# TAMS-Group/bio_ik

Hardware: AMD Instinct MI355X
Metric: IK solves/sec (pop=128, 7-DOF PoseGoal batch) (higher is better)
Workload: dtype f64

## Files before the change

bio_ik_amd/csrc/bioik_kernels.h:

```cpp
#pragma once
#include <type_traits>

#include "bioik_device.h"


#ifndef BIOIK_CANDIDATE_BOUND
#define BIOIK_CANDIDATE_BOUND BIOIK_SINCOS_DOMAIN
#endif
#ifndef BIOIK_COOP_WALKS
#define BIOIK_COOP_WALKS 1
#endif

struct LdsLayout {
    int seed, par, pop, sol, prefix, state, clip, xcol, slots, g_first, g_stride, total;
    int xn, gv, frames, tips, delta, base, grad, red, sec, order, bc;
    int xm, xp, dv, fc;
    int fitp;
    int help;
};
BIOIK_HD LdsLayout make_layout(int n_ops, int V, int P, int T, int n_slots, int nthreads, int lambda, int has_secondary, int child_cols = 1,
                               int groups = 1, int slot_sets = 1, int fit_park = 0, int fc_in_pop = 0, int helped = 0, int bounded = 0) {
    LdsLayout L;
    const int m = n_ops > 0 ? n_ops : 1;
    int o = 0;
// ... 624 lines not shown
        }
    }
    template <class Fn>
    BIOIK_DEV double group_value(bool glead, int gtid, double* s_bc, Fn&& fn) {
        double v = 0.0;
        if (glead) v = fn();
        if (G > 64) {
            if (gtid == 0) s_bc[0] = v;
            wg_barrier();
            v = s_bc[0];
            wg_barrier();
        }
        return v;
    }
    BIOIK_DEV FitCheck group_check(bool glead, int gtid, double* s_bc, const XV& x) {
        const QueryCtx qc{s_seed, s_par};
        FitCheck fc{0.0, 0};
        if (glead) {
            if (BIOIK_COOP_WALKS == 0) fc = exact_fitness_check(pb, x, qc, s_slots, sp.dpos, sp.drot, sp.dtwist, 1, s_prefix);
            else if (G >= 64) fc = exact_fitness_check<64>(pb, x, qc, s_slots, sp.dpos, sp.drot, sp.dtwist, 1, s_prefix);
            else fc = exact_fitness_check<32>(pb, x, qc, s_slots, sp.dpos, sp.drot, sp.dtwist, 1, s_prefix);
        }
        if (G > 64) {
            if (gtid == 0) s_bc[0] = fc.fitness, s_bc[2] = (double)fc.ok;
            wg_barrier();
            fc.fitness = s_bc[0];
            fc.ok = (int)s_bc[2];
            wg_barrier();
        }
        return fc;
    }
    BIOIK_DEV FitCheck wg_check(bool wlead, int tid, const XV& x, double dpos, double drot, double dtwist, int do_check) {
        const QueryCtx qc{s_seed, s_par};
        FitCheck fc{0.0, 0};
        if (wlead) fc = exact_fitness_check<BIOIK_COOP_WALKS ? 64 : 0>(pb, x, qc, s_slots, dpos, drot, dtwist, do_check, s_prefix);
        if (nth > 64) {
            double* const s_wbc = s_state + 16;
            if (tid == 0) s_wbc[0] = fc.fitness, s_wbc[1] = (double)fc.ok;
            wg_barrier();
            fc.fitness = s_wbc[0];
            fc.ok = (int)s_wbc[1];
            wg_barrier();
        }
        return fc;
    }
    BIOIK_DEV SpeciesState species_load(int r) const {
        const double* d = s_state + r * 8;
        return SpeciesState{d[0], d[1], d[2], (int)d[3], (int)d[4], (int)d[5], (int)d[6], (int)d[7]};
    }
    BIOIK_DEV void species_store(int r, const SpeciesState& S) const {
        double* d = s_state + r * 8;
        d[0] = S.fit, d[1] = S.pf0, d[2] = S.pf1, d[3] = (double)S.id, d[4] = (double)S.slot, d[5] = (double)S.cur, d[6] = (double)S.improved, d[7] = (double)S.ok;
    }
    BIOIK_DEV int rank_now(int rank_it) const {
        return (SLIM && groups == 2) ? (HALVES ? p_lane_fresh() >> 5 : (WAVE2 ? p_wave_index() : (g_shift >= 0 ? p_tid_fresh() >> g_shift : p_tid_fresh() / G))) : rank_it;
    }
};

#if defined(BIOIK_PHASE_TIMING)
#define BIOIK_FRAME_PHASE_NAMES(F) auto& ph_t_ = (F).ph_t_; auto& ph_last_ = (F).ph_last_; auto& ph_start_ = (F).ph_start_;
#else
#define BIOIK_FRAME_PHASE_NAMES(F)
#endif
#define BIOIK_FRAME_NAMES(F)                                                                                                                                          \
    typedef typename Frame::PB PB;                                                                                                                                    \
    constexpr bool LEAN = Frame::LEAN, CL = Frame::CL, JOINT = Frame::JOINT, SLIM = Frame::SLIM, DENSE = Frame::DENSE, HELPED = Frame::HELPED, WAVE2 = Frame::WAVE2,   \
                   LIN = Frame::LIN, JH = Frame::JH, HALVES = Frame::HALVES, SELECTS = Frame::SELECTS, columnless = Frame::CL;                                        \
    constexpr int FIXED = Frame::FIXED;                                                                                                                               \
    const SolveArgs& a = (F).a;                                                                                                                                       \
    const DevSolveParams& sp = (F).sp;                                                                                                                                \
    double* const lds = (F).lds;                                                                                                                                      \
    const PB pb = (F).pb;                                                                                                                                             \
    const uint64_t unit = (F).unit, q = (F).q, active_mask = (F).active_mask;                                                                                         \
    const uint32_t key = (F).key;                                                                                                                                     \
    const bool resume = (F).resume, has_sec = (F).has_sec, exact = (F).exact, child_pairs = (F).child_pairs;                                                          \
    const int tid0 = (F).tid0, nth = (F).nth, V = (F).V, P = (F).P, T = (F).T, n_ops = (F).n_ops, D = (F).D, lambda = (F).lambda,                                     \
              n_cols = (F).n_cols, groups = (F).groups, G = (F).G, g_shift = (F).g_shift;                                                                             \
    const int M = n_ops > 0 ? n_ops : 1;                                                                                                                              \
    const int SP = 2 * 2 * 2 * M;                                                                                                   \
    const int BF = 4 * M;                                                             \
    const int carry_n = carry_doubles(n_ops);                                                                        \
    const LdsLayout& L = (F).L;                                                                                                                                       \
    double* const s_seed = (F).s_seed;                                                                                                                                \
    double* const s_par = (F).s_par;                                                                                                                                  \
    double* const s_pop = (F).s_pop;                                                                                                                                  \
    double* const s_sol = (F).s_sol;                                                                                                                                  \
    double* const s_prefix = (F).s_prefix;                                                                                                                            \
    double* const s_state = (F).s_state;                                                                                                                              \
    double* const s_slots = (F).s_slots;                                                                                                                              \
    double* const s_clip = (F).s_clip;                                                                                                                                \
    double* const s_wbc = s_state + 16;                                                                                          \
    double* const s_solst = s_state + 20;                                                                   \
    double* const s_deadline = s_state + 22;                   \
    const QueryCtx qc{s_seed, s_par};                                                                                                                                 \
    auto wg_barrier = [&]() { (F).wg_barrier(); };                                                                                                                    \
    auto species_load = [&](int r_) { return (F).species_load(r_); };                                                                                                 \
    auto species_store = [&](int r_, const SpeciesState& S_) { (F).species_store(r_, S_); };                                                                          \
    auto my_resident = [&]() { return (F).my_resident(); };                                                                                                           \
    (void)wg_barrier, (void)species_load, (void)species_store, (void)my_resident;                                               \
    BIOIK_FRAME_PHASE_NAMES(F)
template <class Frame>
BIOIK_DEV bool solve_setup(Frame& F, uint64_t unit_in) {
    typedef typename Frame::PB PB;
    constexpr bool LEAN = Frame::LEAN, CL = Frame::CL, SLIM = Frame::SLIM, DENSE = Frame::DENSE, HELPED = Frame::HELPED, WAVE2 = Frame::WAVE2, LIN = Frame::LIN, JH = Frame::JH, HALVES = Frame::HALVES;
    constexpr bool columnless = CL;
    constexpr int FIXED = Frame::FIXED;
// ... 564 lines not shown
    } else if (!JOINT && columnless) {
        for (int r = gtid; r < n_eval; r += G) {
            const int c = has_sec ? s_order[r] : r;
            const auto cx = make_child_x(pb, key, ctr1, (uint32_t)c + 2u, p0g, p0d, p1d);
            PHASE_MARK(PH_REPRODUCE);
            const double f = exact ? eval_exact_primary(pb, cx, qc, s_slots, s_prefix) : eval_linear_primary(pb, cx, qc, lm);
            PHASE_MARK(PH_FITNESS);
            offer(f, r + 2);
        }
    } else {
        for (int r = gtid, j = 0; r < n_eval; r += G, j++) {
            int c = has_sec ? s_order[r] : r;
            double* xc = stored ? xcol + (size_t)j * M * nth : xcol;
            const XV xv{xc, nth};
            reproduce_child(pb, key, ctr1, (uint32_t)c + 2u, p0g, p0d, p1d, xc, nth, nullptr, 0);
            PHASE_MARK(PH_REPRODUCE);
            double f = exact ? eval_exact_primary(pb, xv, qc, s_slots, s_prefix) : eval_linear_primary(pb, xv, qc, lm);
            PHASE_MARK(PH_FITNESS);
            offer(f, r + 2);
        }
    }
}

template <class Frame>
BIOIK_DEV void solve_select_and_copy(Frame& F, SpeciesState& S, double*& popS, int rank_it, int step, int gen, uint32_t ctr1, int n_eval, double& b1f, int& b1p, double& b2f, int& b2p) {
    BIOIK_FRAME_NAMES(F);
    auto rank_now = [&]() { return F.rank_now(rank_it); };
    BIOIK_LANE_SCOPE;
    const double* cb = popS + S.cur * BF;
    const double *p0g = cb, *p0d = cb + M, *p1d = cb + 3 * M;
    const bool stored = !columnless && n_cols * G >= lambda && (LEAN || pb->n_quat == 0);
    auto offer = [&](double f, int pos) { top2_insert(b1f, b1p, b2f, b2p, f, pos); };
    auto coarse_parked = [&](int gt) {
        if constexpr (SLIM && CL) {
            if (const int tie_bits = a.preselect >> 8) {
                double* const s_fq = gbase + L.fitp;
                for (int r = gt; r < n_eval; r += G) {
                    unsigned long long v;
                    __builtin_memcpy(&v, &s_fq[r], 8);
                    v &= ~((1ull << tie_bits) - 1ull);
                    __builtin_memcpy(&s_fq[r], &v, 8);
                }
                group_sync(G);
            }
        }
    };
    if constexpr (SLIM) S = species_load(rank_now()), popS = s_pop + S.slot * SP, cb = popS + S.cur * BF, p0g = cb, p0d = cb + M, p1d = cb + 3 * M;
    const uint32_t ctr1w = SLIM ? rng_ctr1((uint32_t)step * 16u + (uint32_t)gen, (uint32_t)S.id, RNG_REPRODUCE) : ctr1;
    if constexpr (DENSE || JH) coarse_parked(gtid);
    if constexpr (DENSE || JH) {
        const double* const s_fit2 = gbase + L.fitp;
        const int drop = a.sort_key_drop;
        unsigned long long k1 = ~0ull, k2 = ~0ull;
        for (int r = gtid; r < n_eval; r += G) {
            const unsigned long long k = sort_key(s_fit2[r], r + 2, drop);
            const bool w1 = k < k1, w2 = k < k2;
            k2 = w1 ? k1 : (w2 ? k : k2);
            k1 = w1 ? k : k1;
        }
        const unsigned long long B1 = half_min_u64(k1);
        const unsigned long long B2 = half_min_u64(k1 == B1 ? k2 : k1);
        int shares = 0;
        for (int r = gtid; r < n_eval; r += G) shares += ((sort_key(s_fit2[r], r + 2, drop) ^ B2) >> drop) == 0ull ? 1 : 0;
        const unsigned long long one = p_ballot(shares > 0), more = p_ballot(shares > 1);
        const uint32_t mine = grp ? (uint32_t)(one >> 32) : (uint32_t)one;
        const bool in_doubt = B2 != ~0ull && ((mine & (mine - 1u)) != 0u);
        if (p_ballot(in_doubt) == 0ull && more == 0ull) {
            b1p = (int)(B1 & 1023ull), b1f = s_fit2[b1p - 2];
            if (B2 != ~0ull) b2p = (int)(B2 & 1023ull), b2f = s_fit2[b2p - 2];
        } else {
            for (int r = gtid; r < n_eval; r += G) offer(s_fit2[r], r + 2);
            top2_wave(b1f, b1p, b2f, b2p, G);
        }
    } else {
        top2_wave(b1f, b1p, b2f, b2p, G);
    }
    PHASE_MARK(PH_SEL_TOP2);
    top2_xwave(b1f, b1p, b2f, b2p, s_red, gtid, G);
    PHASE_MARK(PH_SEL_XWAVE);
    if constexpr (SELECTS) {
        if (has_sec) {
            double* const s_fv = gbase + L.fitp;
            int t1 = 0, t2 = 0;
            for (int r = gtid; r < n_eval; r += G) {
                const double v = s_fv[r];
                t1 += v == b1f ? 1 : 0, t2 += v == b2f ? 1 : 0;
            }
            const unsigned long long gm = G >= 64 ? ~0ull : 0xffffffffull << (tid & 32);
            const unsigned long long o1 = p_ballot(t1 > 0) & gm, o2 = p_ballot(t2 > 0) & gm;
            const bool tie = (p_ballot(t1 > 1 || t2 > 1) & gm) != 0ull || (o1 & (o1 - 1ull)) != 0ull || (o2 & (o2 - 1ull)) != 0ull || (b2p != 0x7fffffff && b2f == S.pf0);
            if (p_ballot(tie) != 0ull) {
                auto stable_first = [&](double fwant, int skip, double& wf, int& wc) -> int {
                    double bs = P_INF;
                    int bc = 0x7fffffff, br = 0x7fffffff;
                    for (int r = gtid; r < n_eval; r += G) {
                        if (!(s_fv[r] == fwant) || r == skip) continue;
                        const int c = s_order[r];
                        const double sec = secondary_fitness<true>(pb, make_child_x(pb, key, ctr1w, (uint32_t)c + 2u, p0g, p0d, p1d), qc);
                        if (sec < bs || (sec == bs && c < bc)) bs = sec, bc = c, br = r;
                    }
                    double w2f = P_INF;
                    int w2c = 0x7fffffff;
                    wf = bs, wc = bc;
                    top2_wave(wf, wc, w2f, w2c, G);
                    const unsigned long long own = p_ballot(bc == wc && bc != 0x7fffffff) & gm;
                    const int src = own != 0ull ? __builtin_ctzll(own) : (tid & 63);
                    const int rr = p_shfl(br, src);
                    return own != 0ull ? rr : 0x7fffffff;
                };
                double e1, e2;
                int c1, c2;
                const int r1 = stable_first(b1f, -1, e1, c1);
                const int r2 = stable_first(b2f, r1, e2, c2);
                if (tie && r1 != 0x7fffffff) {
                    b1p = r1 + 2;
                    if (b2p != 0x7fffffff && r2 != 0x7fffffff) {
                        b2p = r2 + 2;
                        const bool first_is_first = e1 < e2 || (e1 == e2 && c1 < c2);
                        if (first_is_first != (r1 < r2)) {
                            if (gtid == 0) {
                                const int ca = s_order[r1], cb2 = s_order[r2];
                                const double fa = s_fv[r1], fb = s_fv[r2];
                                s_order[r1] = cb2, s_order[r2] = ca, s_fv[r1] = fb, s_fv[r2] = fa;
                            }
                            b1p = r2 + 2, b2p = r1 + 2;
                        }
                    }
                }
                group_sync(G);
            }
        }
    }
    Cand first{S.pf0, 0, 0};
    if (cand_better(S.pf1, 1, first.f, first.pos)) first = Cand{S.pf1, 1, 1};
    if (cand_better(b1f, b1p, first.f, first.pos)) first = Cand{b1f, b1p, b1p};
    const double c2f = (b1p == first.id) ? b2f : b1f;
    const int c2p = (b1p == first.id) ? b2p : b1p;
    Cand second{P_INF, 0x7fffffff, -1};
    if (first.id != 0) second = Cand{S.pf0, first.pos, 0};
    if (first.id != 1 && (second.id < 0 || cand_better(S.pf1, 1, second.f, second.pos))) second = Cand{S.pf1, 1, 1};
    if (second.id < 0 || cand_better(c2f, c2p, second.f, second.pos)) second = Cand{c2f, c2p, c2p};
    double* nb = popS + (S.cur ^ 1) * BF;
    const bool both_at_once = G >= 64 || M <= 16;
    for (int pass = 0; pass < (both_at_once ? 1 : 2); pass++) {
        BIOIK_LANE_SCOPE;
        if (gtid >= 64) break;
        const int i = G >= 64 ? gtid >> 5 : (both_at_once ? gtid >> 4 : pass), k0 = G >= 64 || !both_at_once ? gtid & 31 : gtid & 15;
        const int id = i == 0 ? first.id : second.id;
        double* dst = nb + i * 2 * M;
        if (id < 2) {
            const double* src = cb + id * 2 * M;
            if (k0 < M) dst[k0] = src[k0], dst[M + k0] = src[M + k0];
            if (M > 32 && k0 + 32 < M) dst[k0 + 32] = src[k0 + 32], dst[M + k0 + 32] = src[M + k0 + 32];
        } else if (stored) {
            BIOIK_FP_STRICT
            const int r = id - 2;
            const int c = has_sec ? s_order[r] : r;
            const double fmix = (((uint32_t)c + 2u) % 2u == 0u) ? 0.2 : 0.0;
            const int r_col = (G & (G - 1)) == 0 ? r >> (31 - __builtin_clz((unsigned)G)) : r / G, r_lane = r - r_col * G;
            const double* src = (lds + L.xcol) + (size_t)r_col * M * nth + (grp * G + r_lane);
            auto take = [&](int k) {
                double gene = src[(size_t)k * nth];
                double mom = 0.0;
                if ((active_mask >> k) & 1ull) {
                    double parent_gradient = p0d[k] * (1.0 - fmix) + p1d[k] * fmix;
                    mom = parent_gradient * (1.0 - 0.3) + (gene - p0g[k]) * 0.3;
                }
                dst[k] = gene, dst[M + k] = mom;
            };
            if (k0 < n_ops) take(k0);
            if (n_ops > 32 && k0 + 32 < n_ops) take(k0 + 32);
        } else if (LEAN) {
            BIOIK_FP_STRICT
            const int c = has_sec ? s_order[id - 2] : id - 2;
            const ChildX<PB> cx = make_child_x(pb, key, ctr1w, (uint32_t)c + 2u, p0g, p0d, p1d);
            auto derive = [&](int k) {
                const double gene = cx.template value<false>(k);
                double mom = 0.0;
                if ((active_mask >> k) & 1ull) {
                    const double parent_gradient = p0d[k] * (1.0 - cx.fmix) + p1d[k] * cx.fmix;
                    mom = parent_gradient * (1.0 - 0.3) + (gene - p0g[k]) * 0.3;
                }
                dst[k] = gene, dst[M + k] = mom;
            };
            if (k0 < n_ops) derive(k0);
            if (n_ops > 32 && k0 + 32 < n_ops) derive(k0 + 32);
        } else if (k0 == 0) {
            int c = has_sec ? s_order[id - 2] : id - 2;
            reproduce_child(pb, key, ctr1, (uint32_t)c + 2u, p0g, p0d, p1d, dst, 1, dst + M, 1);
        }
    }
    S.cur ^= 1;
    S.pf0 = first.f;
    S.pf1 = second.f;
    if constexpr (SLIM)
        if (gtid == 0) species_store(rank_now(), S);
    group_sync(G);
    PHASE_MARK(PH_SEL_COPY);
    group_sync(G);
    PHASE_MARK(PH_SEL_BAR);
}

template <class Frame>
BIOIK_DEV void solve_generation(Frame& F, SpeciesState& S, double*& popS, int rank_it, int step, int gen) {
    BIOIK_FRAME_NAMES(F);
    auto rank_now = [&]() { return F.rank_now(rank_it); };
    BIOIK_LANE_SCOPE;
    if constexpr (SLIM) S = species_load(rank_now()), popS = s_pop + S.slot * SP;
    const double* cb = popS + S.cur * BF;
    const double *p0g = cb, *p0d = cb + M, *p1d = cb + 3 * M;
    const uint32_t gctr = (uint32_t)step * 16u + (uint32_t)gen;
    const uint32_t ctr1 = rng_ctr1(gctr, (uint32_t)S.id, RNG_REPRODUCE);
    int n_eval = lambda;
    uint64_t inside_mask = 0ull;
    if constexpr (DENSE || WAVE2 || JH) {
        double* const pgt = popS + (S.cur ^ 1) * BF;
        bool inside = false;
        for (int k = gtid; k < n_ops; k += G) {
            const double d0 = p0d[k], d1 = p1d[k];
            const double pg0 = child_parent_gradient(d0, d1, 0), pg1 = child_parent_gradient(d0, d1, 1);
            pgt[k] = pg0, pgt[M + k] = pg1;
            if constexpr (WAVE2)
                inside = pb->ops[k].gene >= 0 && !op_unbounded(pb, k) && avoid_limits_surely_free(p0g[k], pg0, pg1, op_limit<LIM_VMIN>(pb, k), op_limit<LIM_VMAX>(pb, k), op_limit<LIM_SPAN>(pb, k));
        }
        if constexpr (WAVE2) inside_mask = has_sec ? p_ballot(inside) : 0ull;
        group_sync(G);
    }
    if (has_sec) solve_preselect(F, S, popS, step, gen, ctr1, inside_mask, n_eval);
    double b1f = P_INF, b2f = P_INF;
    int b1p = 0x7fffffff, b2p = 0x7fffffff;
    solve_walks(F, S, popS, rank_it, step, gen, ctr1, n_eval, b1f, b1p, b2f, b2p);
    solve_select_and_copy(F, S, popS, rank_it, step, gen, ctr1, n_eval, b1f, b1p, b2f, b2p);
}

template <class Frame>
BIOIK_DEV void solve_memetic(Frame& F, SpeciesState& S, double*& popS, int rank_it, int step) {
    BIOIK_FRAME_NAMES(F);
    auto rank_now = [&]() { return F.rank_now(rank_it); };
    if constexpr (SLIM) S = species_load(rank_now()), popS = s_pop + S.slot * SP;
    if (sp.memetic) {
        BIOIK_LANE_SCOPE;
        double* el = popS + S.cur * BF;
        const XV xe{el, 1};
        if (exact) build_approximator<BIOIK_COOP_WALKS>(pb, xe, s_slots, s_frames, s_tips, s_delta, s_base, gtid, G, s_prefix);
        PHASE_MARK(PH_MEM_APPROX);
        if (gtid < 64) {
            const int Gw = G < 64 ? G : 64;
            double dp = 0.0000001;
            {
                uint32_t o0, o1;
                philox2x32_10(key, rng_ctr0(0, 0), rng_ctr1((uint32_t)step * 16u, (uint32_t)S.id, RNG_MEMETIC_SIGN), o0, o1);
                if (rng_uniform(o0, o1) < 0.5) dp = -dp;
            }
            const bool by_op = pb_flavour<PB>::general ? pb->genes_follow_ops != 0 : true;
            const int cnt = by_op ? n_ops : D;
            const int my_op = gtid < D ? pb->op_of_gene[gtid] : -1;
            double* s_gop = s_gv;
            const int FB = 8 * T;
            double* s_x4 = s_xn;
            double* s_ex = s_bc;
            auto chains = [&](const double* d0, double* f0, const double* d1, double* f1) {
                for (int idx = gtid; idx < FB; idx += Gw) {
                    const int t = idx >> 3, c = idx & 7;
                    if (c == 7) continue;
                    double a0 = s_tips[t * 7 + c], a1 = a0;
                    const double* dl = s_delta + (size_t)t * n_ops * 7 + c;
                    for (int g0 = 0; g0 < cnt; g0 += 4) {
                        double d[4], v0[4], v1[4];
#pragma unroll
                        for (int j = 0; j < 4; j++) {
                            const int i2 = g0 + j < cnt ? g0 + j : cnt - 1;
                            const int kk = by_op ? i2 : pb->op_of_gene[i2];
                            const bool pad = g0 + j >= cnt;
                            d[j] = dl[(size_t)kk * 7];
                            v0[j] = pad ? 0.0 : d0[kk];
                            v1[j] = (pad || !d1) ? 0.0 : d1[kk];
                        }
#pragma unroll
                        for (int j = 0; j < 4; j++) {
// ... 32 lines not shown
                        }
                    } else {
                        e = goal_eval<false, PerturbX>(pb, type, pb->secondary[g].var_op, pb->secondary[g].var_seed, qc.par + pb->secondary[g].param_off, zero, xown, qc, pb->secondary[g].pad);
                    }
                    sum += e * pb->secondary[g].weight_sq;
                }
                return sum;
            };
            auto goals_on = [&](const double* fc, int dop, double dstep, const PerturbX& x, double& prim, double& all, bool want_all, const PerturbX& xsh, const double* tm) {
#if !defined(BIOIK_NO_POSE_ONLY)
                if (pb->pose_only) {
                    F7 f = frame_of(fc, 0);
                    if (dstep != 0.0 && dop >= 0) {
                        const double* dl = s_delta + (size_t)dop * 7;
                        f = F7{{BK_FMA(dl[0], dstep, f.p.x), BK_FMA(dl[1], dstep, f.p.y), BK_FMA(dl[2], dstep, f.p.z)},
                               {BK_FMA(dl[3], dstep, f.q.x), BK_FMA(dl[4], dstep, f.q.y), BK_FMA(dl[5], dstep, f.q.z), BK_FMA(dl[6], dstep, f.q.w)}};
                    }
                    const double* P = qc.par + pb->pose_param_off;
                    double e = dist2(f.p, v3(P[0], P[1], P[2]));
                    const Q4 d = Q4{P[3] - f.q.x, P[4] - f.q.y, P[5] - f.q.z, P[6] - f.q.w};
                    const Q4 a = Q4{P[3] + f.q.x, P[4] + f.q.y, P[5] + f.q.z, P[6] + f.q.w};
                    const double rs = P[7];
                    e += fmin(qdot(d, d), qdot(a, a)) * (rs * rs);
                    prim = all = e * pb->pose_weight_sq;
                    return;
                }
#endif
                double acc = 0.0;
                V3 bal = v3(0.0, 0.0, 0.0);
                auto tip_frame = [&](int t) -> F7 {
                    F7 f = frame_of(fc, t);
                    if (dstep != 0.0) {
                        double d[7] = {0.0, 0.0, 0.0, 0.0, 0.0, 0.0, 0.0};
                        if (dop >= 0) {
                            const double* dl = s_delta + ((size_t)t * n_ops + dop) * 7;
                            for (int c = 0; c < 7; c++) d[c] = dl[c];
                        }
                        f = F7{{BK_FMA(d[0], dstep, f.p.x), BK_FMA(d[1], dstep, f.p.y), BK_FMA(d[2], dstep, f.p.z)},
                               {BK_FMA(d[3], dstep, f.q.x), BK_FMA(d[4], dstep, f.q.y), BK_FMA(d[5], dstep, f.q.z), BK_FMA(d[6], dstep, f.q.w)}};
                    }
                    return f;
                };
                for (int t = 0; t < T; t++) {
                    const F7 f = tip_frame(t);
                    acc = tip_goals(pb, t, f, x, qc, acc, tip_frame);
                    balance_tip(pb, t, f, bal);
                }
                acc = nonlink_primary(pb, x, qc, acc);
                acc += balance_cost(pb, bal, qc);
                prim = acc;
                if constexpr (DENSE) all = acc + 0.0;
                else all = want_all ? acc + secondary_shared(x, xsh, tm) : acc;
            };
            for (int k = gtid; k < n_ops; k += Gw) s_gop[k] = 0.0;
            const bool odd = gtid & 1;
            bool descending = true;
            double f2p = 0.0, fa = 0.0;
            for (int it = 0; it < 8 && descending; it++) {
                PHASE_COUNT(PH_N_MEM_ITER);
                double fnorm = 0.0;
                bool nan_gene = false;
                for (int round = it == 0 ? 0 : 1; round < 3; round++) {
                    double* dv0 = s_dv + (round == 0 ? 0 : round == 1 ? 1 : 3) * M;
                    double* fc0 = (L.fc >= 0 ? s_fc : popS + (S.cur ^ 1) * BF) + (round == 0 ? 0 : round == 1 ? 1 : 3) * FB;
                    if (round == 0) {
                        for (int k = gtid; k < n_ops; k += Gw) dv0[k] = ((active_mask >> k) & 1ull) ? el[k] - s_base[k] : 0.0;
                    } else if (round == 1) {
                        double sum = dp * dp;
                        for (int i = 0; i < D; i++) sum += fabs(s_grad[i]);
                        fnorm = 1.0 / sum * dp;
                        PHASE_MARK(PH_MEM_NORM);
                        for (int k = gtid; k < n_ops; k += Gw) {
                            const double e = el[k], g = s_gop[k] * fnorm, b = s_base[k];
                            const bool on = (active_mask >> k) & 1ull;
                            const double xm = e - g, xp = e + g;
                            s_xm[k] = xm, s_xp[k] = xp;
                            dv0[k] = on ? xm - b : 0.0;
                            dv0[M + k] = on ? xp - b : 0.0;
                        }
                    } else {
                        const double f1 = s_ex[2], f3 = s_ex[3], f2 = fa;
                        double step_size;
                        if (sp.memetic == 'q') {
                            double v1 = f2 - f1, v2 = f3 - f2;
                            double v = (v1 + v2) * 0.5, aa = v1 - v2;
                            step_size = v / aa;
                        } else {
                            double cost_diff = (f3 - f1) * 0.5;
                            step_size = -(f2 / cost_diff);
                        }
                        bool nan_here = false;
                        for (int k = gtid; k < n_ops; k += Gw) {
                            const double e = el[k], gv = s_gop[k] * fnorm;
                            const bool on = (active_mask >> k) & 1ull;
                            const double raw = e + gv * step_size;
                            const bool is_nan = on && !(raw == raw);
                            const double x4 = (on && !is_nan) ? fmin(fmax(raw, s_clip[k]), s_clip[M + k]) : e;
                            nan_here = nan_here || is_nan || (on && fabs(x4) >= BIOIK_CANDIDATE_BOUND);
                            s_x4[k] = x4;
                            dv0[k] = on ? x4 - s_base[k] : 0.0;
                        }
                        nan_gene = (p_ballot(nan_here) & (G >= 64 ? ~0ull : 0xffffffffull << (tid & 32))) != 0ull;
                    }
                    p_wave_sync();
                    PHASE_MARK(PH_MEM_SUPPORT_COLS);
                    chains(dv0, fc0, round == 1 ? dv0 + M : nullptr, fc0 + FB);
                    p_wave_sync();
                    double vprim, vall;
                    const bool grad_round = round != 1;
                    const PerturbX xq{round == 0 ? el : (round == 2 ? s_x4 : (odd ? s_xp : s_xm)), grad_round ? my_op : -1, grad_round ? dp : 0.0};
                    const PerturbX xs{round == 0 ? el : (round == 2 ? s_x4 : s_xm), grad_round ? my_op : -1, grad_round ? dp : 0.0, round == 1 ? s_xp : nullptr};
                    goals_on(fc0 + ((round == 1 && odd) ? FB : 0), grad_round ? my_op : -1, grad_round ? dp : 0.0, xq, vprim, vall, true, xs,
                             s_tm + ((round == 1 && odd) ? 3 * M : 0));
                    PHASE_MARK(PH_MEM_SUPPORT_EVAL);
                    if (round == 0) {
                        if (gtid == D) s_ex[0] = vprim, s_ex[1] = vall;
                        p_wave_sync();
                        f2p = s_ex[0], fa = s_ex[1];
                        if (my_op >= 0) {
                            s_grad[gtid] = vall - fa;
                            s_gop[my_op] = vall - fa;
                        }
                        p_wave_sync();
                        PHASE_MARK(PH_MEM_GRAD);
                    } else if (round == 1) {
                        if (gtid < 2) s_ex[2 + gtid] = vall;
                        p_wave_sync();
                    } else {
                        if (gtid == D) s_ex[0] = vprim, s_ex[1] = vall;
                        p_wave_sync();
                        const double cprim = s_ex[0], call = s_ex[1];
                        const bool accept = !nan_gene && cprim < f2p;
                        if (G >= 64 ? !accept : p_ballot(accept) == 0ull) descending = false;
                        if (accept) {
                            for (int k = gtid; k < n_ops; k += Gw) el[k] = s_x4[k];
                            f2p = cprim, fa = call;
                            if (my_op >= 0) {
                                s_grad[gtid] = vall - call;
                                s_gop[my_op] = vall - call;
                            }
                        }
                        p_wave_sync();
                        PHASE_MARK(PH_MEM_ACCEPT);
                    }
                }
            }
        }
        group_sync(G);
        PHASE_MARK(PH_MEM_TAIL);
    }
}

template <class Frame>
BIOIK_DEV void solve_rank(Frame& F, SpeciesState& S, double* popS, int rank_it) {
    BIOIK_FRAME_NAMES(F);
    auto rank_now = [&]() { return F.rank_now(rank_it); };
    auto group_check = [&](bool glead_, int gtid_, double* s_bc_, const XV& x_) { return F.group_check(glead_, gtid_, s_bc_, x_); };
    {
        BIOIK_LANE_SCOPE;
        const double* cb = popS + S.cur * BF;
        const FitCheck fc = group_check(glead, gtid, s_bc, XV{cb, 1});
        S.improved = (fc.fitness != S.fit) ? 1 : 0;
        S.fit = fc.fitness;
        S.pf0 = fc.fitness;
        S.ok = fc.ok;
        PHASE_MARK(PH_RANK);
    }
    {
        BIOIK_LANE_SCOPE;
        if (gtid == 0) species_store(rank_now(), S);
    }
}

template <class Frame>
BIOIK_DEV bool solve_species_and_checks(Frame& F, int step) {
    BIOIK_FRAME_NAMES(F);
    int& steps = F.steps;
    bool &success = F.success, &expired = F.expired, &overtaken_out = F.overtaken_out, &drained = F.drained, &lost = F.lost;
    double& final_fit = F.final_fit;
    const int step_first = F.step_first, step_end = F.step_end;
    auto wg_check = [&](bool wlead_, int tid_, const XV& x_, double dpos_, double drot_, double dtwist_, int do_check_) { return F.wg_check(wlead_, tid_, x_, dpos_, drot_, dtwist_, do_check_); };
    wg_barrier();
    BIOIK_LANE_SCOPE;

    SpeciesState A = species_load(0), B = species_load(1);
    if (B.fit < A.fit) {
        SpeciesState tmp = A;
        A = B;
        B = tmp;
    }
    {
        uint32_t o0, o1;
        philox2x32_10(key, rng_ctr0(0, 0), rng_ctr1((uint32_t)step * 16u, (uint32_t)B.id, RNG_WIPEOUT), o0, o1);
        bool wipe = rng_uniform(o0, o1) < 0.1;
        wipe = wipe || !B.improved;
        if (sp.no_wipeout) wipe = false;
// ... 369 lines not shown
```

bio_ik_amd/csrc/bioik_platform.h:

```cpp
#pragma once
#include <stdint.h>

#include "bioik_types.h"

#if defined(BIOIK_PLATFORM_HEADER)
#include BIOIK_PLATFORM_HEADER
#else
#include <hip/hip_runtime.h>
#define BIOIK_DEV __device__ __forceinline__
#define BIOIK_CALL __device__ __attribute__((noinline))
typedef __attribute__((address_space(3))) double lds_f64;
typedef const DevProblem __attribute__((address_space(4))) * ProbPtr;
typedef const DevProblemLean __attribute__((address_space(4))) * LeanProbPtr;

BIOIK_DEV int p_tid() { return (int)threadIdx.x; }
BIOIK_DEV int p_nthreads() { return (int)blockDim.x; }
BIOIK_DEV void p_barrier() { __syncthreads(); }
BIOIK_DEV void p_wave_sync() {
    __builtin_amdgcn_fence(__ATOMIC_RELEASE, "wavefront");
    __builtin_amdgcn_wave_barrier();
    __builtin_amdgcn_fence(__ATOMIC_ACQUIRE, "wavefront");
}
template <class T>
BIOIK_DEV T p_shfl(T v, int src_lane) { return __shfl(v, src_lane, 64); }
// ... 165 lines not shown
    if constexpr (pb_bounded<PB>::value) return pb.lim[LIM_UNBOUNDED * pb.m + k] != 0.0;
    else return pb->ops[k].unbounded;
}
template <class PB>
BIOIK_DEV PB pb_with_limits(PB pb, const double*, int) { return pb; }
BIOIK_DEV BoundedProbPtr pb_with_limits(BoundedProbPtr pb, const double* lim, int m) {
    pb.lim = lim, pb.m = m;
    return pb;
}

#if defined(BIOIK_PHASE_TIMING)
#define PHASE_N 24
#define PHASE_SLOTS 28
#define PHASE_DECL unsigned long long ph_t_[PHASE_N] = {0}, ph_last_ = __builtin_readcyclecounter(), ph_start_ = wall_clock64()
#define PHASE_MARK(i)                                          \
    do {                                                       \
        unsigned long long now_ = __builtin_readcyclecounter(); \
        ph_t_[i] += now_ - ph_last_;                           \
        ph_last_ = now_;                                       \
    } while (0)
#define PHASE_COUNT(i) (ph_t_[i] += 1)
#define PHASE_DUMP(ptr, unit)                                                       \
    do {                                                                            \
        if ((ptr) && p_tid() == 0)                                                  \
        {                                                                           \
            for (int i_ = 0; i_ < PHASE_N; i_++) (ptr)[(unit) * PHASE_SLOTS + i_] = ph_t_[i_]; \
            (ptr)[(unit) * PHASE_SLOTS + PHASE_N] = ph_start_;                      \
            (ptr)[(unit) * PHASE_SLOTS + PHASE_N + 1] = wall_clock64();             \
            (ptr)[(unit) * PHASE_SLOTS + PHASE_N + 2] = (unsigned long long)__builtin_amdgcn_s_getreg((31 << 11) | 4) | ((unsigned long long)__builtin_amdgcn_s_getreg((31 << 11) | 20) << 32); \
            (ptr)[(unit) * PHASE_SLOTS + PHASE_N + 3] = 0;                                   \
        }                                                                           \
    } while (0)
#else
#define PHASE_DECL
#define PHASE_MARK(i)
#define PHASE_DUMP(ptr, unit)
#define PHASE_COUNT(i)
#endif
enum { PH_INIT = 0, PH_REPRODUCE = 1, PH_FITNESS = 2, PH_SELECTION = 3, PH_MEMETICS = 4, PH_SPECIES = 5, PH_CHECK = 6, PH_PRESELECT = 7,
       PH_SEL_TOP2 = 8, PH_SEL_XWAVE = 9, PH_SEL_COPY = 10, PH_SEL_BAR = 11, PH_MEM_APPROX = 12, PH_MEM_GRAD = 13, PH_MEM_NORM = 14,
       PH_MEM_LINE = 15, PH_MEM_ACCEPT = 16, PH_MEM_TAIL = 17, PH_RANK = 18, PH_N_MEM_ITER = 19, PH_N_STEPS = 20, PH_LINEARISE = 21,
       PH_MEM_SUPPORT_COLS = 22, PH_MEM_SUPPORT_EVAL = 23, PH_MEM_CANDIDATE = 7  };

#define BIOIK_SINCOS_FN BIOIK_DEV
#include "bioik_sincos.h"
#define BIOIK_FUSED_FN BIOIK_DEV
#include "bioik_fused.h"
BIOIK_DEV void p_sincos(double x, double* s, double* c) { bioik_sincos(x, s, c); }
#if defined(BIOIK_PLATFORM_HEADER)
BIOIK_DEV bool p_none_of_wave(bool pred) { return !pred; }
#else
BIOIK_DEV bool p_none_of_wave(bool pred) { return __builtin_amdgcn_ballot_w64(pred) == 0ull; }
#endif
template <int N>
BIOIK_DEV bool p_sincos_all_small(const double (&h)[N]) {
    bool large = false;
#pragma unroll
    for (int j = 0; j < N; j++) large = large || !(__builtin_fabs(h[j]) <= BIOIK_SINCOS_SMALL);
    return p_none_of_wave(large);
}
template <int N>
BIOIK_DEV void p_sincos_n(const double (&h)[N], double (&sn)[N], double (&cs)[N]) {
    if (p_sincos_all_small<N>(h)) {
#pragma unroll
        for (int j = 0; j < N; j++) bioik_sincos_small(h[j], &sn[j], &cs[j]);
    } else {
#pragma unroll
        for (int j = 0; j < N; j++) p_sincos(h[j], &sn[j], &cs[j]);
    }
}
BIOIK_DEV void p_sincos_voted(double h, double* s, double* c) {
    const double h1[1] = {h};
    double s1[1], c1[1];
    p_sincos_n<1>(h1, s1, c1);
    *s = s1[0], *c = c1[0];
}
#define BIOIK_ACOS_FN BIOIK_DEV
#include "bioik_acos.h"

#define BIOIK_DBL_MAX 1.7976931348623157e308
#define BIOIK_PI 3.14159265358979323846
```

Measured before the change: 1.254 million.

## Hand parent-gradient table from selection copy to next reproduce; keep sort keys in registers

During selection copy, the DENSE path now computes the next generation's parent-gradient table from the momentum values it just wrote, using a cross-row lane swap (permlane16). This lets the following reproduce step skip its own table-building loop, its group barrier, and the species reload. The top-2 key scan now holds sort keys in a small register array when n_eval fits in 4 or 8 strides, so they are not recomputed from LDS. A trailing group barrier is also removed unless phase timing is enabled. This adds coupling between phases and depends on lane-layout assumptions (n_ops <= 16, two rows of 16 lanes).

Result: faster. 1.270 million, median of 4 (+1.3%).

```diff
diff --git a/bio_ik_amd/csrc/bioik_kernels.h b/bio_ik_amd/csrc/bioik_kernels.h
--- a/bio_ik_amd/csrc/bioik_kernels.h
+++ b/bio_ik_amd/csrc/bioik_kernels.h
@@ -700,6 +700,7 @@
         double* d = s_state + r * 8;
         d[0] = S.fit, d[1] = S.pf0, d[2] = S.pf1, d[3] = (double)S.id, d[4] = (double)S.slot, d[5] = (double)S.cur, d[6] = (double)S.improved, d[7] = (double)S.ok;
     }
+    BIOIK_DEV bool table_handed_over(int gen) const { return DENSE && gen > 0 && gen < sp.generations && n_ops <= 16; }
     BIOIK_DEV int rank_now(int rank_it) const {
         return (SLIM && groups == 2) ? (HALVES ? p_lane_fresh() >> 5 : (WAVE2 ? p_wave_index() : (g_shift >= 0 ? p_tid_fresh() >> g_shift : p_tid_fresh() / G))) : rank_it;
     }
@@ -1370,16 +1371,37 @@
         const double* const s_fit2 = gbase + L.fitp;
         const int drop = a.sort_key_drop;
         unsigned long long k1 = ~0ull, k2 = ~0ull;
-        for (int r = gtid; r < n_eval; r += G) {
-            const unsigned long long k = sort_key(s_fit2[r], r + 2, drop);
+        auto rank_key = [&](unsigned long long k) {
             const bool w1 = k < k1, w2 = k < k2;
             k2 = w1 ? k1 : (w2 ? k : k2);
             k1 = w1 ? k : k1;
-        }
-        const unsigned long long B1 = half_min_u64(k1);
-        const unsigned long long B2 = half_min_u64(k1 == B1 ? k2 : k1);
+        };
+        unsigned long long B1, B2;
         int shares = 0;
-        for (int r = gtid; r < n_eval; r += G) shares += ((sort_key(s_fit2[r], r + 2, drop) ^ B2) >> drop) == 0ull ? 1 : 0;
+        auto with_kept_keys = [&](auto kept_n) {
+            constexpr int KEPT = decltype(kept_n)::value;
+            unsigned long long kept[KEPT];
+#pragma unroll
+            for (int j = 0; j < KEPT; j++) {
+                const int r = gtid + j * G;
+                kept[j] = r < n_eval ? sort_key(s_fit2[r], r + 2, drop) : ~0ull;
+                rank_key(kept[j]);
+            }
+            B1 = half_min_u64(k1);
+            B2 = half_min_u64(k1 == B1 ? k2 : k1);
+#pragma unroll
+            for (int j = 0; j < KEPT; j++) shares += gtid + j * G < n_eval && ((kept[j] ^ B2) >> drop) == 0ull ? 1 : 0;
+        };
+        if (DENSE && n_eval <= 4 * G) {
+            with_kept_keys(std::integral_constant<int, 4>());
+        } else if (DENSE && n_eval <= 8 * G) {
+            with_kept_keys(std::integral_constant<int, 8>());
+        } else {
+            for (int r = gtid; r < n_eval; r += G) rank_key(sort_key(s_fit2[r], r + 2, drop));
+            B1 = half_min_u64(k1);
+            B2 = half_min_u64(k1 == B1 ? k2 : k1);
+            for (int r = gtid; r < n_eval; r += G) shares += ((sort_key(s_fit2[r], r + 2, drop) ^ B2) >> drop) == 0ull ? 1 : 0;
+        }
         const unsigned long long one = p_ballot(shares > 0), more = p_ballot(shares > 1);
         const uint32_t mine = grp ? (uint32_t)(one >> 32) : (uint32_t)one;
         const bool in_doubt = B2 != ~0ull && ((mine & (mine - 1u)) != 0u);
@@ -1466,9 +1488,10 @@
         const int i = G >= 64 ? gtid >> 5 : (both_at_once ? gtid >> 4 : pass), k0 = G >= 64 || !both_at_once ? gtid & 31 : gtid & 15;
         const int id = i == 0 ? first.id : second.id;
         double* dst = nb + i * 2 * M;
+        double mom0 = 0.0;
         if (id < 2) {
             const double* src = cb + id * 2 * M;
-            if (k0 < M) dst[k0] = src[k0], dst[M + k0] = src[M + k0];
+            if (k0 < M) dst[k0] = src[k0], dst[M + k0] = mom0 = src[M + k0];
             if (M > 32 && k0 + 32 < M) dst[k0 + 32] = src[k0 + 32], dst[M + k0 + 32] = src[M + k0 + 32];
         } else if (stored) {
             BIOIK_FP_STRICT
@@ -1485,8 +1508,9 @@
                     mom = parent_gradient * (1.0 - 0.3) + (gene - p0g[k]) * 0.3;
                 }
                 dst[k] = gene, dst[M + k] = mom;
+                return mom;
             };
-            if (k0 < n_ops) take(k0);
+            if (k0 < n_ops) mom0 = take(k0);
             if (n_ops > 32 && k0 + 32 < n_ops) take(k0 + 32);
         } else if (LEAN) {
             BIOIK_FP_STRICT
@@ -1500,12 +1524,22 @@
                     mom = parent_gradient * (1.0 - 0.3) + (gene - p0g[k]) * 0.3;
                 }
                 dst[k] = gene, dst[M + k] = mom;
+                return mom;
             };
-            if (k0 < n_ops) derive(k0);
+            if (k0 < n_ops) mom0 = derive(k0);
             if (n_ops > 32 && k0 + 32 < n_ops) derive(k0 + 32);
         } else if (k0 == 0) {
             int c = has_sec ? s_order[id - 2] : id - 2;
             reproduce_child(pb, key, ctr1, (uint32_t)c + 2u, p0g, p0d, p1d, dst, 1, dst + M, 1);
+        }
+        if constexpr (DENSE) {
+            if (F.table_handed_over(gen + 1)) {
+                const double d1 = p_row_up16(mom0);
+                const double pg0 = child_parent_gradient(mom0, d1, 0), pg1 = child_parent_gradient(mom0, d1, 1);
+                p_wave_sync();
+                double* const pgt = popS + S.cur * BF;
+                if (i == 0 && k0 < n_ops) pgt[k0] = pg0, pgt[M + k0] = pg1;
+            }
         }
     }
     S.cur ^= 1;
@@ -1515,7 +1549,9 @@
         if (gtid == 0) species_store(rank_now(), S);
     group_sync(G);
     PHASE_MARK(PH_SEL_COPY);
+#if defined(BIOIK_PHASE_TIMING)
     group_sync(G);
+#endif
     PHASE_MARK(PH_SEL_BAR);
 }
 
@@ -1524,7 +1560,8 @@
     BIOIK_FRAME_NAMES(F);
     auto rank_now = [&]() { return F.rank_now(rank_it); };
     BIOIK_LANE_SCOPE;
-    if constexpr (SLIM) S = species_load(rank_now()), popS = s_pop + S.slot * SP;
+    if constexpr (SLIM)
+        if (!(DENSE && gen > 0)) S = species_load(rank_now()), popS = s_pop + S.slot * SP;
     const double* cb = popS + S.cur * BF;
     const double *p0g = cb, *p0d = cb + M, *p1d = cb + 3 * M;
     const uint32_t gctr = (uint32_t)step * 16u + (uint32_t)gen;
@@ -1534,15 +1571,17 @@
     if constexpr (DENSE || WAVE2 || JH) {
         double* const pgt = popS + (S.cur ^ 1) * BF;
         bool inside = false;
-        for (int k = gtid; k < n_ops; k += G) {
-            const double d0 = p0d[k], d1 = p1d[k];
-            const double pg0 = child_parent_gradient(d0, d1, 0), pg1 = child_parent_gradient(d0, d1, 1);
-            pgt[k] = pg0, pgt[M + k] = pg1;
-            if constexpr (WAVE2)
-                inside = pb->ops[k].gene >= 0 && !op_unbounded(pb, k) && avoid_limits_surely_free(p0g[k], pg0, pg1, op_limit<LIM_VMIN>(pb, k), op_limit<LIM_VMAX>(pb, k), op_limit<LIM_SPAN>(pb, k));
-        }
-        if constexpr (WAVE2) inside_mask = has_sec ? p_ballot(inside) : 0ull;
-        group_sync(G);
+        if (!F.table_handed_over(gen)) {
+            for (int k = gtid; k < n_ops; k += G) {
+                const double d0 = p0d[k], d1 = p1d[k];
+                const double pg0 = child_parent_gradient(d0, d1, 0), pg1 = child_parent_gradient(d0, d1, 1);
+                pgt[k] = pg0, pgt[M + k] = pg1;
+                if constexpr (WAVE2)
+                    inside = pb->ops[k].gene >= 0 && !op_unbounded(pb, k) && avoid_limits_surely_free(p0g[k], pg0, pg1, op_limit<LIM_VMIN>(pb, k), op_limit<LIM_VMAX>(pb, k), op_limit<LIM_SPAN>(pb, k));
+            }
+            if constexpr (WAVE2) inside_mask = has_sec ? p_ballot(inside) : 0ull;
+            group_sync(G);
+        }
     }
     if (has_sec) solve_preselect(F, S, popS, step, gen, ctr1, inside_mask, n_eval);
     double b1f = P_INF, b2f = P_INF;
diff --git a/bio_ik_amd/csrc/bioik_platform.h b/bio_ik_amd/csrc/bioik_platform.h
--- a/bio_ik_amd/csrc/bioik_platform.h
+++ b/bio_ik_amd/csrc/bioik_platform.h
@@ -241,6 +241,16 @@
 #else
 BIOIK_DEV bool p_none_of_wave(bool pred) { return __builtin_amdgcn_ballot_w64(pred) == 0ull; }
 #endif
+#if defined(BIOIK_PLATFORM_HEADER)
+BIOIK_DEV double p_row_up16(double v) { return p_shfl(v, p_lane_fresh() | 16); }
+#else
+BIOIK_DEV int p_row_up16(int v) { return (int)__builtin_amdgcn_permlane16_swap((unsigned int)v, (unsigned int)v, false, false)[1]; }
+BIOIK_DEV double p_row_up16(double v) {
+    const long long b = __builtin_bit_cast(long long, v);
+    const int lo = p_row_up16((int)b), hi = p_row_up16((int)(b >> 32));
+    return __builtin_bit_cast(double, ((long long)hi << 32) | (unsigned int)lo);
+}
+#endif
 template <int N>
 BIOIK_DEV bool p_sincos_all_small(const double (&h)[N]) {
     bool large = false;
```

## Specialize dense memetic descent loop with register-cached per-lane genes and inline chains

Applied to the files above, without the earlier changes.

Adds a DENSE-only path for the memetic gradient descent loop. It keeps each lane's gene value, base, clip bounds and step in registers instead of re-reading LDS, and assumes a 32-wide group with at most two genes per lane. It also replaces the generic chains() call with an inline 4-way unrolled FMA chain whose single- or two-column variant is chosen at compile time. This trims LDS traffic and loop overhead in a hot loop, at the cost of a duplicated code path and possible register pressure. The new path also simplifies the ballot masks and passes xq and an unshifted s_tm to goals_on where the generic path passes xs and an odd-lane offset.

Result: faster. 1.266 million before, 1.306 million after, median of 6 (+3.2%).

```diff
diff --git a/bio_ik_amd/csrc/bioik_kernels.h b/bio_ik_amd/csrc/bioik_kernels.h
--- a/bio_ik_amd/csrc/bioik_kernels.h
+++ b/bio_ik_amd/csrc/bioik_kernels.h
@@ -1681,96 +1681,249 @@
                 if constexpr (DENSE) all = acc + 0.0;
                 else all = want_all ? acc + secondary_shared(x, xsh, tm) : acc;
             };
-            for (int k = gtid; k < n_ops; k += Gw) s_gop[k] = 0.0;
-            const bool odd = gtid & 1;
-            bool descending = true;
-            double f2p = 0.0, fa = 0.0;
-            for (int it = 0; it < 8 && descending; it++) {
-                PHASE_COUNT(PH_N_MEM_ITER);
-                double fnorm = 0.0;
-                bool nan_gene = false;
-                for (int round = it == 0 ? 0 : 1; round < 3; round++) {
-                    double* dv0 = s_dv + (round == 0 ? 0 : round == 1 ? 1 : 3) * M;
-                    double* fc0 = (L.fc >= 0 ? s_fc : popS + (S.cur ^ 1) * BF) + (round == 0 ? 0 : round == 1 ? 1 : 3) * FB;
-                    if (round == 0) {
-                        for (int k = gtid; k < n_ops; k += Gw) dv0[k] = ((active_mask >> k) & 1ull) ? el[k] - s_base[k] : 0.0;
-                    } else if (round == 1) {
-                        double sum = dp * dp;
-                        for (int i = 0; i < D; i++) sum += fabs(s_grad[i]);
-                        fnorm = 1.0 / sum * dp;
-                        PHASE_MARK(PH_MEM_NORM);
-                        for (int k = gtid; k < n_ops; k += Gw) {
-                            const double e = el[k], g = s_gop[k] * fnorm, b = s_base[k];
-                            const bool on = (active_mask >> k) & 1ull;
-                            const double xm = e - g, xp = e + g;
-                            s_xm[k] = xm, s_xp[k] = xp;
-                            dv0[k] = on ? xm - b : 0.0;
-                            dv0[M + k] = on ? xp - b : 0.0;
+            if constexpr (DENSE) {
+                const bool in0 = gtid < n_ops, wide = n_ops > 32, in1 = wide && gtid + 32 < n_ops;
+                const int k1 = gtid + 32;
+                const bool on0 = in0 && ((active_mask >> gtid) & 1ull), on1 = in1 && ((active_mask >> k1) & 1ull);
+                const double base0 = in0 ? s_base[gtid] : 0.0, cmin0 = in0 ? s_clip[gtid] : 0.0, cmax0 = in0 ? s_clip[M + gtid] : 0.0;
+                double e0 = in0 ? el[gtid] : 0.0;
+                double* const fcb = L.fc >= 0 ? s_fc : popS + (S.cur ^ 1) * BF;
+                const int n4 = n_ops & ~3;
+                const bool comp0 = gtid < FB && (gtid & 7) != 7;
+                const double tip0 = comp0 ? s_tips[(gtid >> 3) * 7 + (gtid & 7)] : 0.0;
+                const double* const dl0 = s_delta + ((gtid >> 3) * n_ops * 7 + (gtid & 7));
+                auto chain_of = [&](auto two, const double start, const double* dl, const double* u, double* out) {
+                    constexpr bool TWO = decltype(two)::value;
+                    const double* w = u + M;
+                    double a0 = start, a1 = start;
+                    for (int g = 0; g < n4; g += 4) {
+                        const double d_0 = dl[g * 7], d_1 = dl[g * 7 + 7], d_2 = dl[g * 7 + 14], d_3 = dl[g * 7 + 21];
+                        const double u_0 = u[g], u_1 = u[g + 1], u_2 = u[g + 2], u_3 = u[g + 3];
+                        a0 = BK_FMA(d_0, u_0, a0), a0 = BK_FMA(d_1, u_1, a0), a0 = BK_FMA(d_2, u_2, a0), a0 = BK_FMA(d_3, u_3, a0);
+                        if constexpr (TWO) {
+                            const double w_0 = w[g], w_1 = w[g + 1], w_2 = w[g + 2], w_3 = w[g + 3];
+                            a1 = BK_FMA(d_0, w_0, a1), a1 = BK_FMA(d_1, w_1, a1), a1 = BK_FMA(d_2, w_2, a1), a1 = BK_FMA(d_3, w_3, a1);
                         }
-                    } else {
-                        const double f1 = s_ex[2], f3 = s_ex[3], f2 = fa;
-                        double step_size;
-                        if (sp.memetic == 'q') {
-                            double v1 = f2 - f1, v2 = f3 - f2;
-                            double v = (v1 + v2) * 0.5, aa = v1 - v2;
-                            step_size = v / aa;
+                    }
+                    for (int g = n4; g < n_ops; g++) {
+                        const double d_0 = dl[g * 7];
+                        a0 = BK_FMA(d_0, u[g], a0);
+                        if constexpr (TWO) a1 = BK_FMA(d_0, w[g], a1);
+                    }
+                    out[0] = a0;
+                    if constexpr (TWO) out[FB] = a1;
+                };
+                auto chains_n = [&](auto two, const double* dvp, double* fcp) {
+                    if (comp0) chain_of(two, tip0, dl0, dvp, fcp + gtid);
+                    if (FB > 32)
+                        for (int idx = gtid + 32; idx < FB; idx += 32) {
+                            const int t = idx >> 3, c = idx & 7;
+                            if (c != 7) chain_of(two, s_tips[t * 7 + c], s_delta + (t * n_ops * 7 + c), dvp, fcp + idx);
+                        }
+                };
+                if (in0) s_gop[gtid] = 0.0;
+                if (in1) s_gop[k1] = 0.0;
+                const bool odd = gtid & 1;
+                bool descending = true;
+                double f2p = 0.0, fa = 0.0;
+                for (int it = 0; it < 8 && descending; it++) {
+                    PHASE_COUNT(PH_N_MEM_ITER);
+                    double fnorm = 0.0, g0 = 0.0, x40 = 0.0;
+                    bool nan_gene = false;
+                    for (int round = it == 0 ? 0 : 1; round < 3; round++) {
+                        const int row = round == 0 ? 0 : round == 1 ? 1 : 3;
+                        double* dv0 = s_dv + row * M;
+                        double* fc0 = fcb + row * FB;
+                        if (round == 0) {
+                            if (in0) dv0[gtid] = on0 ? e0 - base0 : 0.0;
+                            if (in1) dv0[k1] = on1 ? el[k1] - s_base[k1] : 0.0;
+                        } else if (round == 1) {
+                            double sum = dp * dp;
+                            const int D4 = D & ~3;
+                            for (int i = 0; i < D4; i += 4) sum += fabs(s_grad[i]), sum += fabs(s_grad[i + 1]), sum += fabs(s_grad[i + 2]), sum += fabs(s_grad[i + 3]);
+                            for (int i = D4; i < D; i++) sum += fabs(s_grad[i]);
+                            fnorm = 1.0 / sum * dp;
+                            PHASE_MARK(PH_MEM_NORM);
+                            if (in0) {
+                                g0 = s_gop[gtid] * fnorm;
+                                const double xm = e0 - g0, xp = e0 + g0;
+                                s_xm[gtid] = xm, s_xp[gtid] = xp;
+                                dv0[gtid] = on0 ? xm - base0 : 0.0;
+                                dv0[M + gtid] = on0 ? xp - base0 : 0.0;
+                            }
+                            if (in1) {
+                                const double e = el[k1], g = s_gop[k1] * fnorm, b = s_base[k1];
+                                const double xm = e - g, xp = e + g;
+                                s_xm[k1] = xm, s_xp[k1] = xp;
+                                dv0[k1] = on1 ? xm - b : 0.0;
+                                dv0[M + k1] = on1 ? xp - b : 0.0;
+                            }
                         } else {
-                            double cost_diff = (f3 - f1) * 0.5;
-                            step_size = -(f2 / cost_diff);
-                        }
-                        bool nan_here = false;
-                        for (int k = gtid; k < n_ops; k += Gw) {
-                            const double e = el[k], gv = s_gop[k] * fnorm;
-                            const bool on = (active_mask >> k) & 1ull;
-                            const double raw = e + gv * step_size;
-                            const bool is_nan = on && !(raw == raw);
-                            const double x4 = (on && !is_nan) ? fmin(fmax(raw, s_clip[k]), s_clip[M + k]) : e;
-                            nan_here = nan_here || is_nan || (on && fabs(x4) >= BIOIK_CANDIDATE_BOUND);
-                            s_x4[k] = x4;
-                            dv0[k] = on ? x4 - s_base[k] : 0.0;
-                        }
-                        nan_gene = (p_ballot(nan_here) & (G >= 64 ? ~0ull : 0xffffffffull << (tid & 32))) != 0ull;
-                    }
-                    p_wave_sync();
-                    PHASE_MARK(PH_MEM_SUPPORT_COLS);
-                    chains(dv0, fc0, round == 1 ? dv0 + M : nullptr, fc0 + FB);
-                    p_wave_sync();
-                    double vprim, vall;
-                    const bool grad_round = round != 1;
-                    const PerturbX xq{round == 0 ? el : (round == 2 ? s_x4 : (odd ? s_xp : s_xm)), grad_round ? my_op : -1, grad_round ? dp : 0.0};
-                    const PerturbX xs{round == 0 ? el : (round == 2 ? s_x4 : s_xm), grad_round ? my_op : -1, grad_round ? dp : 0.0, round == 1 ? s_xp : nullptr};
-                    goals_on(fc0 + ((round == 1 && odd) ? FB : 0), grad_round ? my_op : -1, grad_round ? dp : 0.0, xq, vprim, vall, true, xs,
-                             s_tm + ((round == 1 && odd) ? 3 * M : 0));
-                    PHASE_MARK(PH_MEM_SUPPORT_EVAL);
-                    if (round == 0) {
-                        if (gtid == D) s_ex[0] = vprim, s_ex[1] = vall;
-                        p_wave_sync();
-                        f2p = s_ex[0], fa = s_ex[1];
-                        if (my_op >= 0) {
-                            s_grad[gtid] = vall - fa;
-                            s_gop[my_op] = vall - fa;
+                            const double f1 = s_ex[2], f3 = s_ex[3], f2 = fa;
+                            double step_size;
+                            if (sp.memetic == 'q') {
+                                double v1 = f2 - f1, v2 = f3 - f2;
+                                double v = (v1 + v2) * 0.5, aa = v1 - v2;
+                                step_size = v / aa;
+                            } else {
+                                double cost_diff = (f3 - f1) * 0.5;
+                                step_size = -(f2 / cost_diff);
+                            }
+                            bool nan_here = false;
+                            {
+                                const double raw = e0 + g0 * step_size;
+                                const bool is_nan = on0 && !(raw == raw);
+                                x40 = (on0 && !is_nan) ? p_clamp(raw, cmin0, cmax0) : e0;
+                                nan_here = is_nan || (on0 && fabs(x40) >= BIOIK_CANDIDATE_BOUND);
+                                if (in0) s_x4[gtid] = x40, dv0[gtid] = on0 ? x40 - base0 : 0.0;
+                            }
+                            if (in1) {
+                                const double e = el[k1], gv = s_gop[k1] * fnorm;
+                                const double raw = e + gv * step_size;
+                                const bool is_nan = on1 && !(raw == raw);
+                                const double x4 = (on1 && !is_nan) ? fmin(fmax(raw, s_clip[k1]), s_clip[M + k1]) : e;
+                                nan_here = nan_here || is_nan || (on1 && fabs(x4) >= BIOIK_CANDIDATE_BOUND);
+                                s_x4[k1] = x4;
+                                dv0[k1] = on1 ? x4 - s_base[k1] : 0.0;
+                            }
+                            nan_gene = (p_ballot(nan_here) & (0xffffffffull << (tid & 32))) != 0ull;
                         }
                         p_wave_sync();
-                        PHASE_MARK(PH_MEM_GRAD);
-                    } else if (round == 1) {
-                        if (gtid < 2) s_ex[2 + gtid] = vall;
+                        PHASE_MARK(PH_MEM_SUPPORT_COLS);
+                        if (round == 1) chains_n(std::true_type{}, dv0, fc0);
+                        else chains_n(std::false_type{}, dv0, fc0);
                         p_wave_sync();
-                    } else {
-                        if (gtid == D) s_ex[0] = vprim, s_ex[1] = vall;
-                        p_wave_sync();
-                        const double cprim = s_ex[0], call = s_ex[1];
-                        const bool accept = !nan_gene && cprim < f2p;
-                        if (G >= 64 ? !accept : p_ballot(accept) == 0ull) descending = false;
-                        if (accept) {
-                            for (int k = gtid; k < n_ops; k += Gw) el[k] = s_x4[k];
-                            f2p = cprim, fa = call;
+                        double vprim, vall;
+                        const bool grad_round = round != 1;
+                        const PerturbX xq{round == 0 ? el : (round == 2 ? s_x4 : (odd ? s_xp : s_xm)), grad_round ? my_op : -1, grad_round ? dp : 0.0};
+                        goals_on(fc0 + ((round == 1 && odd) ? FB : 0), grad_round ? my_op : -1, grad_round ? dp : 0.0, xq, vprim, vall, true, xq, s_tm);
+                        PHASE_MARK(PH_MEM_SUPPORT_EVAL);
+                        if (round == 0) {
+                            if (gtid == D) s_ex[0] = vprim, s_ex[1] = vall;
+                            p_wave_sync();
+                            f2p = s_ex[0], fa = s_ex[1];
                             if (my_op >= 0) {
-                                s_grad[gtid] = vall - call;
-                                s_gop[my_op] = vall - call;
+                                s_grad[gtid] = vall - fa;
+                                s_gop[my_op] = vall - fa;
                             }
+                            p_wave_sync();
+                            PHASE_MARK(PH_MEM_GRAD);
+                        } else if (round == 1) {
+                            if (gtid < 2) s_ex[2 + gtid] = vall;
+                            p_wave_sync();
+                        } else {
+                            if (gtid == D) s_ex[0] = vprim, s_ex[1] = vall;
+                            p_wave_sync();
+                            const double cprim = s_ex[0], call = s_ex[1];
+                            const bool accept = !nan_gene && cprim < f2p;
+                            if (p_ballot(accept) == 0ull) descending = false;
+                            if (accept) {
+                                if (in0) el[gtid] = x40;
+                                if (in1) el[k1] = s_x4[k1];
+                                e0 = x40;
+                                f2p = cprim, fa = call;
+                                if (my_op >= 0) {
+                                    s_grad[gtid] = vall - call;
+                                    s_gop[my_op] = vall - call;
+                                }
+                            }
+                            p_wave_sync();
+                            PHASE_MARK(PH_MEM_ACCEPT);
+                        }
+                    }
+                }
+            } else {
+                for (int k = gtid; k < n_ops; k += Gw) s_gop[k] = 0.0;
+                const bool odd = gtid & 1;
+                bool descending = true;
+                double f2p = 0.0, fa = 0.0;
+                for (int it = 0; it < 8 && descending; it++) {
+                    PHASE_COUNT(PH_N_MEM_ITER);
+                    double fnorm = 0.0;
+                    bool nan_gene = false;
+                    for (int round = it == 0 ? 0 : 1; round < 3; round++) {
+                        double* dv0 = s_dv + (round == 0 ? 0 : round == 1 ? 1 : 3) * M;
+                        double* fc0 = (L.fc >= 0 ? s_fc : popS + (S.cur ^ 1) * BF) + (round == 0 ? 0 : round == 1 ? 1 : 3) * FB;
+                        if (round == 0) {
+                            for (int k = gtid; k < n_ops; k += Gw) dv0[k] = ((active_mask >> k) & 1ull) ? el[k] - s_base[k] : 0.0;
+                        } else if (round == 1) {
+                            double sum = dp * dp;
+                            for (int i = 0; i < D; i++) sum += fabs(s_grad[i]);
+                            fnorm = 1.0 / sum * dp;
+                            PHASE_MARK(PH_MEM_NORM);
+                            for (int k = gtid; k < n_ops; k += Gw) {
+                                const double e = el[k], g = s_gop[k] * fnorm, b = s_base[k];
+                                const bool on = (active_mask >> k) & 1ull;
+                                const double xm = e - g, xp = e + g;
+                                s_xm[k] = xm, s_xp[k] = xp;
+                                dv0[k] = on ? xm - b : 0.0;
+                                dv0[M + k] = on ? xp - b : 0.0;
+                            }
+                        } else {
+                            const double f1 = s_ex[2], f3 = s_ex[3], f2 = fa;
+                            double step_size;
+                            if (sp.memetic == 'q') {
+                                double v1 = f2 - f1, v2 = f3 - f2;
+                                double v = (v1 + v2) * 0.5, aa = v1 - v2;
+                                step_size = v / aa;
+                            } else {
+                                double cost_diff = (f3 - f1) * 0.5;
+                                step_size = -(f2 / cost_diff);
+                            }
+                            bool nan_here = false;
+                            for (int k = gtid; k < n_ops; k += Gw) {
+                                const double e = el[k], gv = s_gop[k] * fnorm;
+                                const bool on = (active_mask >> k) & 1ull;
+                                const double raw = e + gv * step_size;
+                                const bool is_nan = on && !(raw == raw);
+                                const double x4 = (on && !is_nan) ? fmin(fmax(raw, s_clip[k]), s_clip[M + k]) : e;
+                                nan_here = nan_here || is_nan || (on && fabs(x4) >= BIOIK_CANDIDATE_BOUND);
+                                s_x4[k] = x4;
+                                dv0[k] = on ? x4 - s_base[k] : 0.0;
+                            }
+                            nan_gene = (p_ballot(nan_here) & (G >= 64 ? ~0ull : 0xffffffffull << (tid & 32))) != 0ull;
                         }
                         p_wave_sync();
-                        PHASE_MARK(PH_MEM_ACCEPT);
+                        PHASE_MARK(PH_MEM_SUPPORT_COLS);
+                        chains(dv0, fc0, round == 1 ? dv0 + M : nullptr, fc0 + FB);
+                        p_wave_sync();
+                        double vprim, vall;
+                        const bool grad_round = round != 1;
+                        const PerturbX xq{round == 0 ? el : (round == 2 ? s_x4 : (odd ? s_xp : s_xm)), grad_round ? my_op : -1, grad_round ? dp : 0.0};
+                        const PerturbX xs{round == 0 ? el : (round == 2 ? s_x4 : s_xm), grad_round ? my_op : -1, grad_round ? dp : 0.0, round == 1 ? s_xp : nullptr};
+                        goals_on(fc0 + ((round == 1 && odd) ? FB : 0), grad_round ? my_op : -1, grad_round ? dp : 0.0, xq, vprim, vall, true, xs,
+                                 s_tm + ((round == 1 && odd) ? 3 * M : 0));
+                        PHASE_MARK(PH_MEM_SUPPORT_EVAL);
+                        if (round == 0) {
+                            if (gtid == D) s_ex[0] = vprim, s_ex[1] = vall;
+                            p_wave_sync();
+                            f2p = s_ex[0], fa = s_ex[1];
+                            if (my_op >= 0) {
+                                s_grad[gtid] = vall - fa;
+                                s_gop[my_op] = vall - fa;
+                            }
+                            p_wave_sync();
+                            PHASE_MARK(PH_MEM_GRAD);
+                        } else if (round == 1) {
+                            if (gtid < 2) s_ex[2 + gtid] = vall;
+                            p_wave_sync();
+                        } else {
+                            if (gtid == D) s_ex[0] = vprim, s_ex[1] = vall;
+                            p_wave_sync();
+                            const double cprim = s_ex[0], call = s_ex[1];
+                            const bool accept = !nan_gene && cprim < f2p;
+                            if (G >= 64 ? !accept : p_ballot(accept) == 0ull) descending = false;
+                            if (accept) {
+                                for (int k = gtid; k < n_ops; k += Gw) el[k] = s_x4[k];
+                                f2p = cprim, fa = call;
+                                if (my_op >= 0) {
+                                    s_grad[gtid] = vall - call;
+                                    s_gop[my_op] = vall - call;
+                                }
+                            }
+                            p_wave_sync();
+                            PHASE_MARK(PH_MEM_ACCEPT);
+                        }
                     }
                 }
             }
```
